# SciSharp/Gym.NET

Measured on AMD Instinct MI355X. Metric: env-steps/sec, higher is better.
Workload: dtype f32

## Files before the change

### gym.net_amd/csrc/envs.hpp

```cpp
#pragma once
#include <hip/hip_runtime.h>
#include <stdint.h>

#include "philox.hpp"

namespace gymnet {


typedef float f2 __attribute__((ext_vector_type(2)));
namespace vm {
__device__ __forceinline__ float splat(float, float v) { return v; }
__device__ __forceinline__ f2 splat(f2, float v) { return f2{v, v}; }
__device__ __forceinline__ float fma(float a, float b, float c) { return fmaf(a, b, c); }
__device__ __forceinline__ f2 fma(f2 a, f2 b, f2 c) { return __builtin_elementwise_fma(a, b, c); }
template <class T> __device__ __forceinline__ T fmak(float k, T b, T c) { return fma(splat(b, k), b, c); }
template <class T> __device__ __forceinline__ T fmac(T a, T b, float k) { return fma(a, b, splat(a, k)); }
}

__device__ __forceinline__ void sincos_quadrant(float s, float c, float n, float &s_out, float &c_out) {
    const uint32_t q = (uint32_t)(int)n;
    const uint32_t q30 = q << 30, q31 = q << 31;
    const bool odd = (int32_t)q31 < 0;
    const float ss = odd ? c : s, cc = odd ? s : c;
    s_out = __uint_as_float(__builtin_amdgcn_bitop3_b32(__float_as_uint(ss), q30, 0x80000000u, 0x78));
    c_out = __uint_as_float(__builtin_amdgcn_bitop3_b32(__float_as_uint(cc), q30 ^ q31, 0x80000000u, 0x78));
}

template <class T>
__device__ __forceinline__ void sincos_bounded(T x, T &s_out, T &c_out) {
    T n;
    const T xs = x * vm::splat(x, 0.636619772367581343f);
    if constexpr (sizeof(T) == sizeof(float)) n = rintf(xs);
    else n = T{rintf(xs.x), rintf(xs.y)};
    T r = vm::fmak(-1.5703125f, n, x);
    r = vm::fmak(-4.837512969970703125e-4f, n, r);
    r = vm::fmak(-7.54978995489188216e-8f, n, r);
    const T z = r * r;
    T ps = vm::fmac(vm::splat(z, -1.9515295891e-4f), z, 8.3321608736e-3f);
    ps = vm::fmac(ps, z, -1.6666654611e-1f);
    const T s = vm::fma(r * z, ps, r);
    T pc = vm::fmac(vm::splat(z, 2.443315711809948e-5f), z, -1.388731625493765e-3f);
    pc = vm::fmac(pc, z, 4.166664568298827e-2f);
    const T c = vm::fma(z * z, pc, vm::fmac(vm::splat(z, -0.5f), z, 1.0f));
    if constexpr (sizeof(T) == sizeof(float)) {
        sincos_quadrant(s, c, n, s_out, c_out);
    } else {
        float s0, c0, s1, c1;
        sincos_quadrant(s.x, c.x, n.x, s0, c0);
        sincos_quadrant(s.y, c.y, n.y, s1, c1);
        s_out = T{s0, s1};
        c_out = T{c0, c1};
    }
}

template <class T>
__device__ __forceinline__ void sincos_small(T x, T &s_out, T &c_out) {
    T n;
    const T xs = x * vm::splat(x, 0.636619772367581343f);
    if constexpr (sizeof(T) == sizeof(float)) n = rintf(xs);
    else n = T{rintf(xs.x), rintf(xs.y)};
    T r = vm::fmak(-0x1.921fap+0f, n, x);
    r = vm::fmak(-0x1.54442ep-20f, n, r);
    const T z = r * r;
    T ps = vm::fmac(vm::splat(z, -1.9515295891e-4f), z, 8.3321608736e-3f);
    ps = vm::fmac(ps, z, -1.6666654611e-1f);
    const T s = vm::fma(r * z, ps, r);
    T pc = vm::fmac(vm::splat(z, 2.443315711809948e-5f), z, -1.388731625493765e-3f);
    pc = vm::fmac(pc, z, 4.166664568298827e-2f);
    pc = vm::fmac(pc, z, -0.5f);
    const T c = vm::fmac(pc, z, 1.0f);
    if constexpr (sizeof(T) == sizeof(float)) {
        sincos_quadrant(s, c, n, s_out, c_out);
    } else {
        float s0, c0, s1, c1;
        sincos_quadrant(s.x, c.x, n.x, s0, c0);
        sincos_quadrant(s.y, c.y, n.y, s1, c1);
        s_out = T{s0, s1};
        c_out = T{c0, c1};
    }
}

constexpr float kSmallAngle = 0.785f;
__device__ __forceinline__ void sincos_tiny(float x, float &s_out, float &c_out) {
    const float z = x * x;
    float ps = fmaf(-1.9515295891e-4f, z, 8.3321608736e-3f);
    ps = fmaf(ps, z, -1.6666654611e-1f);
    s_out = fmaf(x * z, ps, x);
    float pc = fmaf(2.443315711809948e-5f, z, -1.388731625493765e-3f);
    pc = fmaf(pc, z, 4.166664568298827e-2f);
    c_out = fmaf(z * z, pc, fmaf(-0.5f, z, 1.0f));
}

template <bool BOUNDED = false>
__device__ __forceinline__ void sincos_f32(float x, float &s_out, float &c_out) {
    if constexpr (!BOUNDED) {
        if (__builtin_expect(fabsf(x) > 65536.0f, 0)) {
            sincosf(x, &s_out, &c_out);
            return;
        }
    }
    sincos_bounded<float>(x, s_out, c_out);
}
__device__ __forceinline__ float sin_f32(float x) { float s, c; sincos_f32(x, s, c); return s; }
__device__ __forceinline__ float cos_f32(float x) { float s, c; sincos_f32(x, s, c); return c; }

template <typename Dummy = void>
struct DivByTotalMass {
    static constexpr float C = 0.1f + 1.0f;
    static constexpr float ZH = 1.0f / C;
    static constexpr float ZL = (float)(1.0 / (double)C - (double)ZH);
    __device__ __forceinline__ static float apply(float x) { return fmaf(x, ZH, x * ZL); }
};

struct CartPole {
    static constexpr int S = 4;
    static constexpr int O = 4;
    static constexpr bool OBS_ALIASES_STATE = true;
    static constexpr bool HAS_SBD = true;
    static constexpr bool BOX_ACTION = false;
    static constexpr bool PACKED2 = false;
    static constexpr bool PIPE_LANES = false, PIPE_PAIRS = false;
    using Action = int32_t;
    using Real = float;
    static constexpr bool RESET_TAKES_KEY = false;
    static constexpr const char *NAME = "CartPole";
    static constexpr int32_t ACTION_N = 2;

    static constexpr float gravity = 9.8f;
    static constexpr float masspole = 0.1f;
    static constexpr float total_mass = 0.1f + 1.0f;
    static constexpr float length = 0.5f;
    static constexpr float polemass_length = 0.1f * 0.5f;
    static constexpr float force_mag = 10.0f;
    static constexpr float tau = 0.02f;
    static constexpr float theta_threshold = 0.20943951606750488f;
    static constexpr float x_threshold = 2.4f;

    __device__ __forceinline__ static float div_tm(float x) { return DivByTotalMass<>::apply(x); }

    static constexpr bool HAS_SMALL_ANGLE_PATH = true;
    static constexpr int ANGLE_ROW = 2;
    static constexpr float SMALL_ANGLE_BOUND = kSmallAngle;

    template <bool SMALL_ANGLE = false, bool AUTORESET = false>
    __device__ __forceinline__ static void step(float (&s)[S], Action a, float &reward, bool &done) {
        const float x = s[0], x_dot = s[1], theta = s[2], theta_dot = s[3];
        const float s_in[S] = {x, x_dot, theta, theta_dot};
        const float force = (a == 1) ? force_mag : -force_mag;
        float sintheta, costheta;
        if constexpr (SMALL_ANGLE) sincos_tiny(theta, sintheta, costheta);
        else sincos_f32(theta, sintheta, costheta);
        const float temp = div_tm(force + polemass_length * theta_dot * theta_dot * sintheta);
        const float thetaacc = (gravity * sintheta - costheta * temp)
                               / (length * (4.0f / 3.0f - div_tm(masspole * costheta * costheta)));
        const float xacc = temp - div_tm(polemass_length * thetaacc * costheta);
        const float nx = x + tau * x_dot;
        const float nx_dot = x_dot + tau * xacc;
        const float ntheta = theta + tau * theta_dot;
        const float ntheta_dot = theta_dot + tau * thetaacc;
        s[0] = nx; s[1] = nx_dot; s[2] = ntheta; s[3] = ntheta_dot;
        bool term[DONE_TERMS];
        done_terms_of_inputs(s_in, term);
        done = term[0] || term[1];
        reward = 1.0f;
    }

    static constexpr int DONE_TERMS = 2;
    __device__ __forceinline__ static void done_terms_of_inputs(const float (&s)[S], bool (&term)[DONE_TERMS]) {
        const double vx = __builtin_fma((double)tau, (double)s[1], (double)s[0]);
        const double vtheta = __builtin_fma((double)tau, (double)s[3], (double)s[2]);
        term[0] = __builtin_fabs(vx) > (double)x_threshold;
        term[1] = __builtin_fabs(vtheta) > (double)theta_threshold;
    }

    __device__ __forceinline__ static void reset(float (&s)[S], const PhiloxWords &r) {
#pragma unroll
        for (int k = 0; k < 4; ++k) s[k] = -0.05f + 0.1f * u01_24(r.w[k]);
    }

    __device__ __forceinline__ static void observe(const float (&s)[S], float (&o)[O]) {
#pragma unroll
        for (int k = 0; k < 4; ++k) o[k] = s[k];
    }
    __device__ __forceinline__ static void observe_fresh(const float (&s)[S], float (&o)[O]) { observe(s, o); }
    __device__ __forceinline__ static void step_observe(float (&s)[S], Action a, float &reward, bool &done, float (&o)[O]) {
        step(s, a, reward, done);
        observe(s, o);
    }
};

struct Pendulum {
    static constexpr int S = 2;
    static constexpr int O = 3;
    static constexpr bool OBS_ALIASES_STATE = false;
    static constexpr int OBS_ROW_OF_STATE[S] = {-1, 2};
    static constexpr bool HAS_SBD = false;
    static constexpr bool BOX_ACTION = true;
    static constexpr bool PACKED2 = false;
    static constexpr bool PIPE_LANES = false, PIPE_PAIRS = false;
    static constexpr bool HAS_SMALL_ANGLE_PATH = false;
    using Action = float;
    using Real = float;
    static constexpr bool RESET_TAKES_KEY = false;
    static constexpr const char *NAME = "Pendulum";
    static constexpr float ACTION_LOW = -2.0f, ACTION_HIGH = 2.0f;
    static constexpr float PI = 3.14159265358979323846f;

    __device__ __forceinline__ static float fmod_2pi(float a) {
        constexpr float m = 2.0f * PI, inv_m = 1.0f / m;
        const float ax = fabsf(a);
        if (__builtin_expect(!(ax < 4194304.0f * m), 0)) return fmodf(a, m);
        float q = truncf(ax * inv_m);
        float r = fmaf(-q, m, ax);
        q = r < 0.0f ? q - 1.0f : (r >= m ? q + 1.0f : q);
        r = fmaf(-q, m, ax);
        return copysignf(r, a);
    }

    __device__ __forceinline__ static float floored_mod_2pi(float a) {
        float r = fmod_2pi(a);
        if (r < 0.0f) r += 2.0f * PI;
        return r;
    }

    __device__ __forceinline__ static void step(float (&s)[S], Action a, float &reward, bool &done) {
        const float max_speed = 8.0f, max_torque = 2.0f, dt = 0.05f;
        const float th = s[0], thdot = s[1];
        const float u = a < -max_torque ? -max_torque : (a > max_torque ? max_torque : a);
        const float nrm = floored_mod_2pi(th + PI) - PI;
        const float costs = nrm * nrm + 0.1f * (thdot * thdot) + 0.001f * (u * u);
        float newthdot = thdot + (15.0f * sin_f32(th) + 3.0f * u) * dt;
        newthdot = newthdot < -max_speed ? -max_speed : (newthdot > max_speed ? max_speed : newthdot);
        const float newth = th + newthdot * dt;
        s[0] = newth; s[1] = newthdot;
        reward = -costs;
        done = false;
    }

    __device__ __forceinline__ static void reset(float (&s)[S], const PhiloxWords &r) {
        s[0] = -PI + (2.0f * PI) * u01_24(r.w[0]);
        s[1] = -1.0f + 2.0f * u01_24(r.w[1]);
    }

    __device__ __forceinline__ static void observe(const float (&s)[S], float (&o)[O]) {
        float sn, cs;
        sincos_f32(s[0], sn, cs);
        o[0] = cs; o[1] = sn; o[2] = s[1];
    }
    __device__ __forceinline__ static void observe_fresh(const float (&s)[S], float (&o)[O]) { observe(s, o); }
    __device__ __forceinline__ static void step_observe(float (&s)[S], Action a, float &reward, bool &done, float (&o)[O]) {
        step(s, a, reward, done);
        observe(s, o);
    }
};

struct MountainCar {
    static constexpr int S = 2;
    static constexpr int O = 2;
    static constexpr bool OBS_ALIASES_STATE = true;
    static constexpr bool HAS_SBD = false;
    static constexpr bool BOX_ACTION = false;
    static constexpr bool PACKED2 = false;
    static constexpr bool PIPE_LANES = false, PIPE_PAIRS = false;
    static constexpr bool HAS_SMALL_ANGLE_PATH = false;
    using Action = int32_t;
    using Real = float;
    static constexpr bool RESET_TAKES_KEY = false;
    static constexpr const char *NAME = "MountainCar";
    static constexpr int32_t ACTION_N = 3;

    __device__ __forceinline__ static void step(float (&s)[S], Action a, float &reward, bool &done) {
        float p = s[0], v = s[1];
        v += (float)(a - 1) * 0.001f + cos_f32(3.0f * p) * (-0.0025f);
        v = v < -0.07f ? -0.07f : (v > 0.07f ? 0.07f : v);
        p += v;
        p = p < -1.2f ? -1.2f : (p > 0.6f ? 0.6f : p);
        if (p == -1.2f && v < 0.0f) v = 0.0f;
        s[0] = p; s[1] = v;
        reward = -1.0f;
        done = p >= 0.5f && v >= 0.0f;
    }

    __device__ __forceinline__ static void reset(float (&s)[S], const PhiloxWords &r) {
        s[0] = -0.6f + 0.2f * u01_24(r.w[0]);
        s[1] = 0.0f;
    }

    __device__ __forceinline__ static void observe(const float (&s)[S], float (&o)[O]) { o[0] = s[0]; o[1] = s[1]; }
    __device__ __forceinline__ static void observe_fresh(const float (&s)[S], float (&o)[O]) { observe(s, o); }
    __device__ __forceinline__ static void step_observe(float (&s)[S], Action a, float &reward, bool &done, float (&o)[O]) {
        step(s, a, reward, done);
        observe(s, o);
    }
};

struct MountainCarContinuous {
    static constexpr int S = 2;
    static constexpr int O = 2;
    static constexpr bool OBS_ALIASES_STATE = true;
    static constexpr bool HAS_SBD = false;
    static constexpr bool BOX_ACTION = true;
    static constexpr bool PACKED2 = false;
    static constexpr bool PIPE_LANES = false, PIPE_PAIRS = false;
    static constexpr bool HAS_SMALL_ANGLE_PATH = false;
    using Action = float;
    using Real = float;
    static constexpr bool RESET_TAKES_KEY = false;
    static constexpr const char *NAME = "MountainCarContinuous";
    static constexpr float ACTION_LOW = -1.0f, ACTION_HIGH = 1.0f;
    static constexpr float GOAL = 0x1.cccccep-2f;

    __device__ __forceinline__ static void step(float (&s)[S], Action a, float &reward, bool &done) {
        float p = s[0], v = s[1];
        const float force = a < -1.0f ? -1.0f : (a > 1.0f ? 1.0f : a);
        v += force * 0.0015f - 0.0025f * cos_f32(3.0f * p);
        v = v < -0.07f ? -0.07f : (v > 0.07f ? 0.07f : v);
        p += v;
        p = p < -1.2f ? -1.2f : (p > 0.6f ? 0.6f : p);
        if (p == -1.2f && v < 0.0f) v = 0.0f;
// ... 161 lines not shown
```

### gym.net_amd/csrc/step_kernels.hpp

```cpp
#pragma once
#include "kernels.hpp"

#include <cstdio>
#include <type_traits>

#include "lanes.hpp"
#include "philox.hpp"

namespace gymnet {

__device__ __forceinline__ float abs_real(float x) { return fabsf(x); }
__device__ __forceinline__ double abs_real(double x) { return __builtin_fabs(x); }

template <class Env, bool UNIFORM_KEY = false>
__device__ __forceinline__ void draw_reset(typename Env::Real (&s)[Env::S], uint64_t key, uint64_t lane, uint64_t tick) {
    if constexpr (Env::RESET_TAKES_KEY) Env::reset(s, key, lane, tick);
    else Env::reset(s, lane_words<UNIFORM_KEY>(key, lane, tick));
}

template <class Env>
__device__ __forceinline__ constexpr bool state_row_own(int k) {
    if constexpr (Env::OBS_ALIASES_STATE) return true; else return Env::OBS_ROW_OF_STATE[k] < 0;
}
template <class Env>
__device__ __forceinline__ const typename Env::Real *state_row_src(const typename Env::Real *state, int64_t state_stride,
                                                                    const typename Env::Real *obs_in, int64_t obs_stride, int k) {
    if constexpr (Env::OBS_ALIASES_STATE) return state + k * state_stride;
    else return Env::OBS_ROW_OF_STATE[k] < 0 ? state + k * state_stride : obs_in + Env::OBS_ROW_OF_STATE[k] * obs_stride;
}

__device__ __forceinline__ uint32_t wave_shard() {
    return (uint32_t)((((int64_t)blockIdx.x * blockDim.x + threadIdx.x) >> 6) & (kShards - 1));
}

template <int VEC, class Args>
__device__ __forceinline__ void count_after_done(const Args &a, const bool (&after)[VEC]) {
    uint32_t total = 0;
#pragma unroll
    for (int j = 0; j < VEC; ++j) total += (uint32_t)__popcll(__ballot(after[j]));
    if (total && lane_id() == (uint32_t)(__ffsll((unsigned long long)__ballot(1)) - 1))
        atomicAdd(&a.after_done[wave_shard() * kAfterStride], (unsigned long long)total);
}

template <class Env, bool AUTORESET, bool SMALL_ANGLE = false>
__device__ __forceinline__ void advance_sublane(typename Env::Real (&sj)[Env::S], typename Env::Action act, int32_t &sbd, float &rw,
                                                bool &dn, bool &after, bool in_range, typename Env::Real (&oj)[Env::O]) {
    if constexpr (Env::HAS_SMALL_ANGLE_PATH) Env::template step<SMALL_ANGLE, AUTORESET>(sj, act, rw, dn);
    else if constexpr (Env::OBS_ALIASES_STATE) Env::step(sj, act, rw, dn);
    else Env::step_observe(sj, act, rw, dn, oj);
    if constexpr (!AUTORESET && Env::HAS_SBD) {
        if (dn) {
            if (sbd == -1) { sbd = 0; }
            else { after = in_range; sbd += 1; rw = 0.0f; }
        }
    }
}

template <class Env, int VEC>
__device__ __forceinline__ bool wave_angles_small(const typename Env::Real (&s)[Env::S][VEC]) {
    if constexpr (!Env::HAS_SMALL_ANGLE_PATH) return false;
    else {
        bool small = true;
#pragma unroll
        for (int j = 0; j < VEC; ++j) small = small && (abs_real(s[Env::ANGLE_ROW][j]) <= Env::SMALL_ANGLE_BOUND);
        return __ballot(!small) == 0;
    }
}

template <class Env, int VEC, bool AUTORESET, bool GUARD, bool PACK = true>
__device__ __forceinline__ void advance_all(typename Env::Real (&s)[Env::S][VEC], typename Env::Action (&act)[VEC], int32_t (&sbd)[VEC],
                                            float (&rw)[VEC], bool (&dn)[VEC], bool (&after)[VEC], typename Env::Real (&o)[Env::O][VEC],
                                            int64_t i0, int64_t n) {
    constexpr int S = Env::S, O = Env::O;
    using Real = typename Env::Real;
#ifndef GYMNET_PROBE_NO_PACK
    constexpr bool kPack = true;
#else
    constexpr bool kPack = false;
#endif
    if constexpr (Env::PACKED2 && VEC == 2 && kPack && PACK) {
        Env::step_observe_x2(s, act, rw, dn, o);
    } else {
        auto all_sublanes = [&](auto small_tag) {
#pragma unroll
            for (int j = 0; j < VEC; ++j) {
                Real sj[S], oj[O];
#pragma unroll
                for (int k = 0; k < S; ++k) sj[k] = s[k][j];
                advance_sublane<Env, AUTORESET, decltype(small_tag)::value>(sj, act[j], sbd[j], rw[j], dn[j], after[j], !GUARD || i0 + j < n, oj);
#pragma unroll
                for (int k = 0; k < S; ++k) s[k][j] = sj[k];
                if constexpr (!Env::OBS_ALIASES_STATE) {
#pragma unroll
                    for (int k = 0; k < O; ++k) o[k][j] = oj[k];
                }
            }
        };
        if constexpr (Env::HAS_SMALL_ANGLE_PATH) {
            if (wave_angles_small<Env, VEC>(s)) all_sublanes(std::true_type{});
            else all_sublanes(std::false_type{});
        } else {
            all_sublanes(std::false_type{});
        }
    }
}

template <class Env, class = void> struct has_done_of_inputs : std::false_type {};
template <class Env> struct has_done_of_inputs<Env, std::void_t<decltype(&Env::done_terms_of_inputs)>> : std::true_type {};

template <class Env, int VEC, bool AUTORESET>
__device__ __forceinline__ void advance_all_late_done(typename Env::Real (&s)[Env::S][VEC], typename Env::Action (&act)[VEC], float (&rw)[VEC],
                                                      bool (&dn)[VEC], uint64_t (&dmask)[VEC]) {
    constexpr int S = Env::S, O = Env::O;
    using Real = typename Env::Real;
    static_assert(Env::HAS_SMALL_ANGLE_PATH && Env::OBS_ALIASES_STATE && has_done_of_inputs<Env>::value, "see above");
    static_assert(AUTORESET || !Env::HAS_SBD, "the steps_beyond_done rule reads the flag inside the step");
    Real was[S][VEC];
#pragma unroll
    for (int k = 0; k < S; ++k)
#pragma unroll
        for (int j = 0; j < VEC; ++j) was[k][j] = s[k][j];
    auto all_sublanes = [&](auto small_tag) {
#pragma unroll
        for (int j = 0; j < VEC; ++j) {
            Real sj[S], oj[O];
            int32_t sbd_unused = 0;
            bool after_unused = false;
#pragma unroll
            for (int k = 0; k < S; ++k) sj[k] = s[k][j];
            advance_sublane<Env, AUTORESET, decltype(small_tag)::value>(sj, act[j], sbd_unused, rw[j], dn[j], after_unused, true, oj);
#pragma unroll
            for (int k = 0; k < S; ++k) s[k][j] = sj[k];
        }
    };
    if (wave_angles_small<Env, VEC>(s)) all_sublanes(std::true_type{});
    else all_sublanes(std::false_type{});
#pragma unroll
    for (int j = 0; j < VEC; ++j) {
        Real wj[S];
#pragma unroll
        for (int k = 0; k < S; ++k) wj[k] = was[k][j];
        bool term[Env::DONE_TERMS];
        Env::done_terms_of_inputs(wj, term);
        bool any = false;
        uint64_t m = 0;
#pragma unroll
        for (int q = 0; q < Env::DONE_TERMS; ++q) { any = any || term[q]; m |= __builtin_amdgcn_ballot_w64(term[q]); }
        dn[j] = any;
        dmask[j] = m;
    }
}

template <class Env, int VEC, bool LANE_SEEDS>
__device__ __forceinline__ void reset_pending(uint32_t pending, typename Env::Real (&s)[Env::S][VEC], typename Env::Real (&o)[Env::O][VEC],
                                              const StepArgsT<typename Env::Real> &a, int64_t i0, int64_t n, uint64_t tick) {
    constexpr int S = Env::S, O = Env::O;
    using Real = typename Env::Real;
    while (pending) {
        const int j = __ffs(pending) - 1;
        pending &= pending - 1;
        Real sj[S];
        bool drawn = false;
        if constexpr (LANE_SEEDS) {
            if (a.lane_seed) {
                draw_reset<Env, false>(sj, i0 + j < n ? a.lane_seed[i0 + j] : a.seed, a.lane_offset + (uint64_t)(i0 + j), tick);
                drawn = true;
            }
        }
        if (!drawn) draw_reset<Env, true>(sj, a.seed, a.lane_offset + (uint64_t)(i0 + j), tick);
        Real oj[O];
        if constexpr (!Env::OBS_ALIASES_STATE) Env::observe_fresh(sj, oj);
#pragma unroll
        for (int jj = 0; jj < VEC; ++jj) {
            if (jj == j) {
#pragma unroll
                for (int k = 0; k < S; ++k) s[k][jj] = sj[k];
                if constexpr (!Env::OBS_ALIASES_STATE) {
#pragma unroll
                    for (int k = 0; k < O; ++k) o[k][jj] = oj[k];
                }
            }
        }
    }
}

template <class Env>
constexpr bool has_split_reset() { return Env::RESET_TAKES_KEY && Env::OBS_ALIASES_STATE; }

__device__ __forceinline__ PhiloxWords neighbour_words(const PhiloxWords &w) {
    PhiloxWords o;
#pragma unroll
    for (int k = 0; k < 4; ++k) o.w[k] = (uint32_t)__builtin_amdgcn_mov_dpp((int)w.w[k], 0xB1, 0xF, 0xF, true);
    return o;
}

#ifdef GYMNET_PROBE_RESET_MASKED
constexpr bool kResetFullExec = false;
#else
constexpr bool kResetFullExec = true;
#endif

template <class Env>
struct ResetScratch {
    uint32_t slot[64];
    typename Env::Real draw[64][Env::S];
};

__device__ __forceinline__ void wave_lds_fence() {
    __builtin_amdgcn_fence(__ATOMIC_RELEASE, "wavefront");
    __builtin_amdgcn_wave_barrier();
    __builtin_amdgcn_fence(__ATOMIC_ACQUIRE, "wavefront");
}

template <class Env, int VEC, bool LANE_SEEDS>
__device__ __forceinline__ void reset_pending_wave(uint32_t pending, typename Env::Real (&s)[Env::S][VEC], const StepArgsT<typename Env::Real> &a,
                                                   int64_t i0, int64_t n, uint64_t tick, ResetScratch<Env> *sc) {
    constexpr int S = Env::S;
    using Real = typename Env::Real;
    static_assert(Env::OBS_ALIASES_STATE, "the compacted reset hands back the state only");
    const uint32_t lane = lane_id();
    uint32_t rank[VEC];
    uint32_t total = 0;
#pragma unroll
    for (int j = 0; j < VEC; ++j) {
        const uint64_t m = __ballot((pending >> j) & 1u);
        rank[j] = total + __builtin_amdgcn_mbcnt_hi((uint32_t)(m >> 32), __builtin_amdgcn_mbcnt_lo((uint32_t)m, 0u));
        total += (uint32_t)__popcll(m);
    }
    if (total == 0) return;
    const int64_t wave_i0 = i0 - (int64_t)lane * VEC;
    constexpr bool SPLIT = has_split_reset<Env>();
    const uint32_t active = (uint32_t)__popcll(__ballot(1));
    const uint32_t A = SPLIT ? active >> 1 : active;
    if constexpr (SPLIT) {
        if (A == 0) {
            Real o_unused[Env::O][VEC];
            reset_pending<Env, VEC, LANE_SEEDS>(pending, s, o_unused, a, i0, n, tick);
            return;
        }
    }
    for (uint32_t base = 0; base < total; base += A) {
#pragma unroll
        for (int j = 0; j < VEC; ++j)
            if (((pending >> j) & 1u) && rank[j] - base < A) sc->slot[rank[j] - base] = lane * VEC + (uint32_t)j;
        wave_lds_fence();
        if constexpr (SPLIT) {
            const uint32_t r = lane >> 1, call = lane & 1u;
            const bool draws = r < A && r < total - base;
            PhiloxWords w{};
            if (kResetFullExec || draws) {
                const uint32_t sl = sc->slot[draws ? r : 0u];
                const int64_t gl = wave_i0 + (int64_t)sl;
                uint64_t key = a.seed;
                if constexpr (LANE_SEEDS) {
                    if (a.lane_seed && gl < n) key = a.lane_seed[gl];
                }
                w = lane_words(Env::reset_call_key(key, call), a.lane_offset + (uint64_t)gl, tick);
            }
            const PhiloxWords other = neighbour_words(w);
            if ((kResetFullExec || draws) && call == 0) {
                Real sj[S];
                Env::reset_from_words(sj, w, other);
#pragma unroll
                for (int k = 0; k < S; ++k) sc->draw[r][k] = sj[k];
            }
        } else if (kResetFullExec || lane < total - base) {
            const uint32_t sl = sc->slot[lane < total - base ? lane : 0u];
            const int64_t gl = wave_i0 + (int64_t)sl;
            Real sj[S];
            bool drawn = false;
            if constexpr (LANE_SEEDS) {
                if (a.lane_seed) {
                    draw_reset<Env, false>(sj, gl < n ? a.lane_seed[gl] : a.seed, a.lane_offset + (uint64_t)gl, tick);
                    drawn = true;
                }
            }
            if (!drawn) draw_reset<Env, true>(sj, a.seed, a.lane_offset + (uint64_t)gl, tick);
#pragma unroll
            for (int k = 0; k < S; ++k) sc->draw[lane][k] = sj[k];
        }
        wave_lds_fence();
        Real got[VEC][S];
#pragma unroll
        for (int j = 0; j < VEC; ++j) {
            const uint32_t r = rank[j] - base;
#pragma unroll
            for (int k = 0; k < S; ++k) got[j][k] = sc->draw[r < A ? r : 0u][k];
        }
#pragma unroll
        for (int j = 0; j < VEC; ++j) {
            const bool mine = ((pending >> j) & 1u) && rank[j] - base < A;
#pragma unroll
            for (int k = 0; k < S; ++k) s[k][j] = mine ? got[j][k] : s[k][j];
        }
        wave_lds_fence();
    }
}

template <class Env, int VEC, bool LANE_SEEDS>
__device__ __forceinline__ void reset_finished_wave(const bool (&fin)[VEC], const uint64_t (&fmask)[VEC], typename Env::Real (&s)[Env::S][VEC], const StepArgsT<typename Env::Real> &a,
                                                    int64_t i0, int64_t wave_i0, int64_t n, uint64_t tick, ResetScratch<Env> *sc) {
    constexpr int S = Env::S;
    using Real = typename Env::Real;
    static_assert(Env::OBS_ALIASES_STATE && !has_split_reset<Env>(), "one-call resets that hand back the state only");
    const uint32_t lane = lane_id();
    uint32_t rank[VEC];
    uint32_t total = 0;
#pragma unroll
    for (int j = 0; j < VEC; ++j) {
        const uint64_t m = fmask[j];
        rank[j] = total + __builtin_amdgcn_mbcnt_hi((uint32_t)(m >> 32), __builtin_amdgcn_mbcnt_lo((uint32_t)m, 0u));
        total += (uint32_t)__popcll(m);
    }
    if (__builtin_expect(total == 0 || total > 64u || __ballot(1) != ~0ull, 0)) {
        if (total != 0) {
            uint32_t pending = 0;
#pragma unroll
            for (int j = 0; j < VEC; ++j) pending |= fin[j] ? (1u << j) : 0u;
            reset_pending_wave<Env, VEC, LANE_SEEDS>(pending, s, a, i0, n, tick, sc);
        }
        return;
    }
#pragma unroll
    for (int j = 0; j < VEC; ++j)
        if (fin[j]) sc->slot[rank[j]] = lane * VEC + (uint32_t)j;
    wave_lds_fence();
    {
        const uint32_t sl = sc->slot[lane < total ? lane : 0u];
        const int64_t gl = wave_i0 + (int64_t)sl;
        Real sj[S];
        bool drawn = false;
        if constexpr (LANE_SEEDS) {
            if (a.lane_seed) {
                draw_reset<Env, false>(sj, gl < n ? a.lane_seed[gl] : a.seed, a.lane_offset + (uint64_t)gl, tick);
                drawn = true;
            }
        }
        if (!drawn) draw_reset<Env, true>(sj, a.seed, a.lane_offset + (uint64_t)gl, tick);
#pragma unroll
        for (int k = 0; k < S; ++k) sc->draw[lane][k] = sj[k];
    }
    wave_lds_fence();
    Real got[VEC][S];
#pragma unroll
    for (int j = 0; j < VEC; ++j) {
#pragma unroll
        for (int k = 0; k < S; ++k) got[j][k] = sc->draw[rank[j] & 63u][k];
    }
#pragma unroll
    for (int j = 0; j < VEC; ++j) {
#pragma unroll
        for (int k = 0; k < S; ++k) s[k][j] = fin[j] ? got[j][k] : s[k][j];
    }
    wave_lds_fence();
}

template <int VEC>
__device__ __forceinline__ uint32_t rank_finished(const bool (&finished)[VEC], uint32_t (&off)[VEC]) {
    uint32_t total = 0;
#pragma unroll
    for (int j = 0; j < VEC; ++j) {
        const uint64_t m = __ballot(finished[j]);
        off[j] = total + __builtin_amdgcn_mbcnt_hi((uint32_t)(m >> 32), __builtin_amdgcn_mbcnt_lo((uint32_t)m, 0u));
        total += (uint32_t)__popcll(m);
    }
    return total;
}

template <class Env, int VEC>
__device__ __forceinline__ void append_done_records(const StepArgsT<typename Env::Real> &a, const bool (&finished)[VEC], int64_t i0,
                                                    const typename Env::Real (&s)[Env::S][VEC], const typename Env::Real (&o)[Env::O][VEC],
                                                    const float (&fin_ret)[VEC], const int32_t (&fin_len)[VEC], bool stats) {
    constexpr int S = Env::S, O = Env::O;
    const uint32_t lane = lane_id();
    uint32_t off[VEC];
    const uint32_t total = rank_finished<VEC>(finished, off);
    if (total) {
        const int leader = __ffsll((unsigned long long)__ballot(1)) - 1;
        const uint32_t shard = wave_shard();
        uint32_t base = 0;
        if ((int)lane == leader)
            base = atomicAdd(&a.done_count2[a.cparity * (kShards * kCountStride) + shard * kCountStride], total);
        base = __shfl(base, leader);
        const int64_t seg0 = (int64_t)shard * a.done_cap;
#pragma unroll
        for (int j = 0; j < VEC; ++j) {
            if (!finished[j]) continue;
            const int64_t pos = seg0 + base + off[j];
            a.done_list[pos] = (int32_t)(i0 + j);
            if (stats) { a.rec_ret[pos] = fin_ret[j]; a.rec_len[pos] = fin_len[j]; }
            if (a.rec_obs) {
#pragma unroll
                for (int k = 0; k < O; ++k)
                    a.rec_obs[((int64_t)shard * O + k) * a.done_cap + base + off[j]] = Env::OBS_ALIASES_STATE ? s[k < S ? k : 0][j] : o[k][j];
            }
        }
    }
}

template <class R>
__device__ __forceinline__ StepArgsT<R> hot_step_args(R *state, const void *action, int64_t n, int64_t state_stride, uint64_t *tick2, float *reward,
                                                      int32_t parity, const StepArgsT<R> &rest) {
    StepArgsT<R> a = rest;
    a.state = state; a.action = action; a.n = n; a.state_stride = state_stride; a.tick2 = tick2; a.reward = reward; a.parity = parity;
    return a;
}

template <class Env, int VEC>
struct LaneInputs {
    typename Env::Real s[Env::S][VEC];
    typename Env::Action act[VEC];
    int32_t sbd[VEC];
};

template <bool NT, class T>
__device__ __forceinline__ T load_elem(const T *p) { if constexpr (NT) return __builtin_nontemporal_load(p); else return *p; }

template <class T, int VEC, bool NT>
__device__ __forceinline__ void load_row_clamped(const T *__restrict__ p, int64_t i0, int64_t n, T (&v)[VEC]) {
#pragma unroll
    for (int j = 0; j < VEC; ++j) v[j] = load_elem<NT>(p + (i0 + j < n ? i0 + j : n - 1));
}

template <class Env, int VEC, bool AUTORESET, int NT>
__device__ __forceinline__ void load_inputs_clamped(const StepArgsT<typename Env::Real> &a, const int64_t i0, LaneInputs<Env, VEC> &in) {
    constexpr bool NT_SL = (NT & 1) != 0, NT_A = (NT & 4) != 0;
#pragma unroll
    for (int k = 0; k < Env::S; ++k)
        load_row_clamped<typename Env::Real, VEC, NT_SL>(state_row_src<Env>(a.state, a.state_stride, a.obs_in, a.obs_stride, k), i0, a.n, in.s[k]);
    if constexpr (Env::BOX_ACTION) load_row_clamped<float, VEC, NT_A>(static_cast<const float *>(a.action), i0, a.n, in.act);
    else load_row_clamped<int32_t, VEC, NT_A>(static_cast<const int32_t *>(a.action), i0, a.n, in.act);
#pragma unroll
    for (int j = 0; j < VEC; ++j) in.sbd[j] = 0;
    if constexpr (!AUTORESET && Env::HAS_SBD) load_row_clamped<int32_t, VEC, NT_SL>(a.sbd, i0, a.n, in.sbd);
}

template <class Env, int VEC, bool AUTORESET, int NT, bool GUARD>
__device__ __forceinline__ void load_inputs(const StepArgsT<typename Env::Real> &a, const int64_t i0, LaneInputs<Env, VEC> &in) {
    constexpr bool NT_SL = (NT & 1) != 0, NT_A = (NT & 4) != 0;
    if constexpr (GUARD) { load_inputs_clamped<Env, VEC, AUTORESET, NT>(a, i0, in); return; }
    const int64_t n = a.n;
#pragma unroll
    for (int k = 0; k < Env::S; ++k)
        load_row<typename Env::Real, VEC, NT_SL, GUARD>(state_row_src<Env>(a.state, a.state_stride, a.obs_in, a.obs_stride, k), i0, n, in.s[k]);
    if constexpr (Env::BOX_ACTION) load_f32<VEC, NT_A, GUARD>(static_cast<const float *>(a.action), i0, n, in.act);
    else load_i32<VEC, NT_A, GUARD>(static_cast<const int32_t *>(a.action), i0, n, in.act);
#pragma unroll
    for (int j = 0; j < VEC; ++j) in.sbd[j] = 0;
    if constexpr (!AUTORESET && Env::HAS_SBD) load_i32<VEC, NT_SL, GUARD>(a.sbd, i0, n, in.sbd);
}

template <class Env, int VEC, bool AUTORESET, bool EXTRAS, int NT, bool GUARD, int RESETF = 0, bool PACK = true>
__device__ __forceinline__ void advance_and_store(const StepArgsT<typename Env::Real> &a, const int64_t i0, const uint64_t tick,
                                                  LaneInputs<Env, VEC> &in, ResetScratch<Env> *sc = nullptr) {
    constexpr int S = Env::S, O = Env::O;
    using Real = typename Env::Real;
    constexpr bool NT_SS = (NT & 2) != 0, NT_O = (NT & 8) != 0;
    const int64_t n = a.n;
    Real (&s)[S][VEC] = in.s;
    typename Env::Action (&act)[VEC] = in.act;
    int32_t (&sbd)[VEC] = in.sbd;

    constexpr bool NT_SL = (NT & 1) != 0;
    float ep_ret[VEC], fin_ret[VEC];
    int32_t ep_len[VEC], fin_len[VEC];
    bool stats = false;
    if constexpr (EXTRAS) {
        stats = a.ep_ret != nullptr;
        if (stats) {
            if constexpr (GUARD) { load_row_clamped<float, VEC, NT_SL>(a.ep_ret, i0, n, ep_ret); load_row_clamped<int32_t, VEC, NT_SL>(a.ep_len, i0, n, ep_len); }
            else { load_f32<VEC, NT_SL, false>(a.ep_ret, i0, n, ep_ret); load_i32<VEC, NT_SL, false>(a.ep_len, i0, n, ep_len); }
        }
#pragma unroll
        for (int j = 0; j < VEC; ++j) { fin_ret[j] = 0.0f; fin_len[j] = 0; }
    }

    float reward[VEC];
    uint8_t done[VEC];
    bool finished[VEC];
    bool after[VEC];
#pragma unroll
    for (int j = 0; j < VEC; ++j) after[j] = false;
    Real o[O][VEC];
    uint32_t pending = 0;

    float rwv[VEC];
    bool dnv[VEC];
    advance_all<Env, VEC, AUTORESET, GUARD, PACK>(s, act, sbd, rwv, dnv, after, o, i0, n);

#pragma unroll
    for (int j = 0; j < VEC; ++j) {
        const float rw = rwv[j];
        uint8_t db = dnv[j] ? 1 : 0;
        if constexpr (EXTRAS) {
            if (stats) {
                ep_ret[j] += rw;
                ep_len[j] += 1;
                if (a.max_episode_steps > 0 && ep_len[j] >= a.max_episode_steps) db |= 2;
            }
        }
        const bool fin = db != 0;
        finished[j] = fin && (!GUARD || i0 + j < n);
        done[j] = db;
        reward[j] = rw;

        if constexpr (EXTRAS) {
            if (fin && a.final_obs && (!GUARD || i0 + j < n)) {
#pragma unroll
                for (int k = 0; k < O; ++k) a.final_obs[k * n + i0 + j] = Env::OBS_ALIASES_STATE ? s[k < S ? k : 0][j] : o[k][j];
            }
            if (stats && fin && (!GUARD || i0 + j < n)) {
                fin_ret[j] = ep_ret[j];
                fin_len[j] = ep_len[j];
                if (a.fin_ret) { a.fin_ret[i0 + j] = ep_ret[j]; a.fin_len[i0 + j] = ep_len[j]; }
                if constexpr (AUTORESET) { ep_ret[j] = 0.0f; ep_len[j] = 0; }
            }
        }

        if constexpr (AUTORESET) pending |= fin ? (1u << j) : 0u;
    }

    if constexpr (!AUTORESET && Env::HAS_SBD) count_after_done<VEC>(a, after);

    store_f32<VEC, NT_O, GUARD>(a.reward, i0, n, reward);
    store_u8<VEC, NT_O, GUARD>(a.done, i0, n, done);

    if constexpr (EXTRAS) {
        if (a.done_list) append_done_records<Env, VEC>(a, finished, i0, s, o, fin_ret, fin_len, stats);
    }

    if constexpr (AUTORESET && RESETF == 1) reset_pending_wave<Env, VEC, EXTRAS>(pending, s, a, i0, n, tick, sc);
    else if constexpr (AUTORESET) reset_pending<Env, VEC, EXTRAS>(pending, s, o, a, i0, n, tick);

#pragma unroll
    for (int k = 0; k < S; ++k)
        if (state_row_own<Env>(k)) store_row<Real, VEC, NT_SS, GUARD>(a.state_out + k * a.state_stride, i0, n, s[k]);
    if constexpr (!Env::OBS_ALIASES_STATE) {
#pragma unroll
        for (int k = 0; k < O; ++k) store_row<Real, VEC, NT_SS, GUARD>(a.obs + k * a.obs_stride, i0, n, o[k]);
    }
    if constexpr (!AUTORESET && Env::HAS_SBD) store_i32<VEC, NT_SS, GUARD>(a.sbd, i0, n, sbd);

    if constexpr (EXTRAS) {
        if (stats) { store_f32<VEC, NT_SS, GUARD>(a.ep_ret, i0, n, ep_ret); store_i32<VEC, NT_SS, GUARD>(a.ep_len, i0, n, ep_len); }
    }
}

template <class Env, int VEC, bool AUTORESET, bool EXTRAS, int NT, bool GUARD, int RESETF = 0>
__device__ __forceinline__ void step_body(const StepArgsT<typename Env::Real> &a, const int64_t i0, const uint64_t tick, ResetScratch<Env> *sc = nullptr) {
    LaneInputs<Env, VEC> in;
    load_inputs<Env, VEC, AUTORESET, NT, GUARD>(a, i0, in);
    advance_and_store<Env, VEC, AUTORESET, EXTRAS, NT, GUARD, RESETF>(a, i0, tick, in, sc);
}

template <class Env, bool AUTORESET, bool EXTRAS>
constexpr bool has_full_workgroup_body() {
    return AUTORESET && !EXTRAS && Env::HAS_SMALL_ANGLE_PATH && Env::OBS_ALIASES_STATE && !has_split_reset<Env>() && has_done_of_inputs<Env>::value;
}

template <class T>
__device__ __forceinline__ T *wg_row(T *row, const WgLanes &wg) { return wave_uniform(row + wg.first); }

template <class Env, int VEC, int NT, int RESETF>
__device__ __forceinline__ void step_body_wg(const StepArgsT<typename Env::Real> &a, const WgLanes wg, const uint64_t tick, ResetScratch<Env> *sc) {
    constexpr int S = Env::S;
    using Real = typename Env::Real;
    constexpr bool NT_SL = (NT & 1) != 0, NT_SS = (NT & 2) != 0, NT_A = (NT & 4) != 0, NT_O = (NT & 8) != 0;
    static_assert(!Env::BOX_ACTION && Env::OBS_ALIASES_STATE, "a discrete-action env whose observation is its state");
    const int64_t i0 = wg.first + (int64_t)wg.local;

    Real s[S][VEC];
    typename Env::Action act[VEC];
#pragma unroll
    for (int k = 0; k < S; ++k) load_row_wg<Real, VEC, NT_SL>(wg_row(static_cast<const Real *>(a.state) + k * a.state_stride, wg), wg.local, s[k]);
    load_row_wg<int32_t, VEC, NT_A>(wg_row(static_cast<const int32_t *>(a.action), wg), wg.local, act);

    float reward[VEC];
    bool finished[VEC];
    uint64_t fmask[VEC];
    advance_all_late_done<Env, VEC, true>(s, act, reward, finished, fmask);

    {
        const uint32_t local = reissued(wg.local);
        store_row_wg<float, VEC, NT_O>(wg_row(a.reward, wg), local, reward);
        uint32_t w = 0;
#pragma unroll
        for (int j = 0; j < VEC; ++j) w |= finished[j] ? (1u << (8 * j)) : 0u;
        store_done_word_wg<VEC, NT_O>(wg_row(a.done, wg), local, w);
    }

    if constexpr (RESETF == 1) {
        reset_finished_wave<Env, VEC, false>(finished, fmask, s, a, i0, wg.first + (int64_t)__builtin_amdgcn_readfirstlane(wg.local), a.n, tick, sc);
    } else {
        uint32_t pending = 0;
#pragma unroll
        for (int j = 0; j < VEC; ++j) pending |= finished[j] ? (1u << j) : 0u;
        Real o_unused[Env::O][VEC];
        reset_pending<Env, VEC, false>(pending, s, o_unused, a, i0, a.n, tick);
    }

    const uint32_t local = reissued(wg.local);
#pragma unroll
    for (int k = 0; k < S; ++k) store_row_wg<Real, VEC, NT_SS>(wg_row(a.state_out + k * a.state_stride, wg), local, s[k]);
}

template <class Env>
struct LaneOutputs { typename Env::Real s[Env::S], o[Env::O]; float reward; uint8_t done; int32_t sbd; };

template <class Env, bool AUTORESET>
__device__ __forceinline__ void compute_lane(const StepArgsT<typename Env::Real> &a, int64_t i, uint64_t tick, LaneInputs<Env, 1> &in,
                                             LaneOutputs<Env> &out) {
    constexpr int S = Env::S, O = Env::O;
    typename Env::Real o[O][1];
    float rw[1];
    bool dn[1], after[1] = {false};
    advance_all<Env, 1, AUTORESET, false>(in.s, in.act, in.sbd, rw, dn, after, o, i, a.n);
    if constexpr (!AUTORESET && Env::HAS_SBD) count_after_done<1>(a, after);
    if constexpr (AUTORESET) reset_pending<Env, 1, false>(dn[0] ? 1u : 0u, in.s, o, a, i, a.n, tick);
#pragma unroll
    for (int k = 0; k < S; ++k) out.s[k] = in.s[k][0];
#pragma unroll
    for (int k = 0; k < O; ++k) out.o[k] = o[k][0];
    out.reward = rw[0]; out.done = dn[0] ? 1 : 0; out.sbd = in.sbd[0];
}

template <class Env, bool AUTORESET, int NT>
__device__ __forceinline__ void store_lane(const StepArgsT<typename Env::Real> &a, int64_t i, const LaneOutputs<Env> &out) {
    constexpr bool NT_SS = (NT & 2) != 0, NT_O = (NT & 8) != 0;
    auto st = [](auto *p, auto v, bool nt) { if (nt) __builtin_nontemporal_store(v, p); else *p = v; };
    st(a.reward + i, out.reward, NT_O);
    if constexpr (NT_O) __builtin_nontemporal_store(out.done, a.done + i); else a.done[i] = out.done;
#pragma unroll
    for (int k = 0; k < Env::S; ++k)
        if (state_row_own<Env>(k)) st(a.state_out + k * a.state_stride + i, out.s[k], NT_SS);
    if constexpr (!Env::OBS_ALIASES_STATE) {
#pragma unroll
        for (int k = 0; k < Env::O; ++k) st(a.obs + k * a.obs_stride + i, out.o[k], NT_SS);
    }
    if constexpr (!AUTORESET && Env::HAS_SBD) a.sbd[i] = out.sbd;
}

template <class Env, int ITEMS, bool AUTORESET, int NT>
__global__ __launch_bounds__(256) void step_kernel_pipe(typename Env::Real *state, const void *action, int64_t n, int64_t state_stride, uint64_t *tick2,
                                                        float *reward, int32_t block, int32_t parity, const StepArgsT<typename Env::Real> rest) {
    const StepArgsT<typename Env::Real> a = hot_step_args(state, action, n, state_stride, tick2, reward, parity, rest);
    const uint64_t tick = a.tick2[a.parity];
    if (blockIdx.x == 0 && threadIdx.x == 0) a.tick2[a.parity ^ 1] = tick + 1;
    const int64_t T = (int64_t)gridDim.x * block;
    const int64_t i = (int64_t)blockIdx.x * block + threadIdx.x;
    LaneInputs<Env, 1> in[ITEMS];
#pragma unroll
    for (int k = 0; k < ITEMS; ++k) {
        const int64_t idx = i + k * T;
        load_inputs<Env, 1, AUTORESET, NT, false>(a, idx < a.n ? idx : a.n - 1, in[k]);
    }
#pragma unroll
    for (int k = 0; k < ITEMS; ++k) {
        LaneOutputs<Env> out;
        if (k == 0) {
#pragma unroll
            for (int c = 0; c < Env::S; ++c) asm volatile("" : "+v"(in[0].s[c][0]));
            asm volatile("" : "+v"(in[0].act[0]));
        }
        compute_lane<Env, AUTORESET>(a, i + k * T, tick, in[k], out);
        if (k == 0) {
#pragma unroll
            for (int kk = 1; kk < ITEMS; ++kk) {
#pragma unroll
                for (int c = 0; c < Env::S; ++c) asm volatile("" : "+v"(in[kk].s[c][0]), "+v"(out.s[Env::S - 1]));
                asm volatile("" : "+v"(in[kk].act[0]), "+v"(out.reward));
            }
        }
        if (i + k * T < a.n) store_lane<Env, AUTORESET, NT>(a, i + k * T, out);
    }
}

template <class Env>
struct DeferScratch {
    uint32_t slot[32];
    typename Env::Real draw[32][Env::S];
};

template <class Env, int PAIRS, class StateOf>
__device__ __forceinline__ void reset_group_deferred(uint32_t pending, StateOf s, const StepArgsT<typename Env::Real> &a, int64_t t_wave0,
                                                     int64_t T, int first_pair, uint64_t tick, DeferScratch<Env> *sc) {
    static_assert(Env::RESET_CALLS == 2 && 2 * PAIRS <= 8, "two lanes per reset; the slot word keeps 3 bits for the sub-lane position");
    constexpr int Q = 2 * PAIRS, S = Env::S;
    using Real = typename Env::Real;
    const uint32_t lane = lane_id();
    uint32_t rank[Q];
    uint32_t total = 0;
#pragma unroll
    for (int q = 0; q < Q; ++q) {
        const uint64_t m = __ballot((pending >> q) & 1u);
        rank[q] = total + __builtin_amdgcn_mbcnt_hi((uint32_t)(m >> 32), __builtin_amdgcn_mbcnt_lo((uint32_t)m, 0u));
        total += (uint32_t)__popcll(m);
    }
    for (uint32_t base = 0; base < total; base += 32) {
#pragma unroll
        for (int q = 0; q < Q; ++q)
            if (((pending >> q) & 1u) && rank[q] - base < 32u) sc->slot[rank[q] - base] = lane * 8u + (uint32_t)q;
        wave_lds_fence();
        const uint32_t r = lane >> 1, call = lane & 1u;
        const bool draws = r < total - base;
        PhiloxWords w{};
        if (kResetFullExec || draws) {
            const uint32_t sl = sc->slot[draws ? r : 0u];
            const uint32_t owner = sl >> 3, q = sl & 7u;
            const int64_t gl = ((t_wave0 + owner) + (int64_t)(first_pair + (int)(q >> 1)) * T) * 2 + (q & 1u);
            w = lane_words(Env::reset_call_key(a.seed, call), a.lane_offset + (uint64_t)gl, tick);
        }
        const PhiloxWords other = neighbour_words(w);
        if ((kResetFullExec || draws) && call == 0) {
            Real sj[S];
            Env::reset_from_words(sj, w, other);
#pragma unroll
            for (int k = 0; k < S; ++k) sc->draw[r][k] = sj[k];
        }
        wave_lds_fence();
        Real got[Q][S];
#pragma unroll
        for (int q = 0; q < Q; ++q) {
            const uint32_t rr = rank[q] - base;
#pragma unroll
            for (int k = 0; k < S; ++k) got[q][k] = sc->draw[rr < 32u ? rr : 0u][k];
        }
#pragma unroll
        for (int q = 0; q < Q; ++q) {
            const bool mine = ((pending >> q) & 1u) && rank[q] - base < 32u;
            Real (&sq)[S][2] = s(q / 2);
#pragma unroll
            for (int k = 0; k < S; ++k) sq[k][q % 2] = mine ? got[q][k] : sq[k][q % 2];
        }
        wave_lds_fence();
    }
}

template <class Env, int ITEMS, int NT, bool GUARD>
__device__ __forceinline__ void pipe2_split_body(const StepArgsT<typename Env::Real> &a, int64_t t, int64_t T, uint64_t tick, DeferScratch<Env> *sc) {
    using Real = typename Env::Real;
    constexpr bool NT_SS = (NT & 2) != 0, NT_O = (NT & 8) != 0;
    LaneInputs<Env, 2> in[ITEMS];
#pragma unroll
    for (int k = 0; k < ITEMS; ++k) {
        load_inputs<Env, 2, true, NT, GUARD>(a, (t + k * T) * 2, in[k]);
    }
    uint32_t pending = 0;
#pragma unroll
    for (int k = 0; k < ITEMS; ++k) {
        if (k == 0) {
#pragma unroll
// ... 858 lines not shown
```

Measured before the change: 161.6 billion.

## Split CartPole step into action-independent pre and post phases, draw resets ahead

Splits the CartPole step into an action-independent pre phase (sincos, divisor, next positions) and a cheap action-dependent post phase. Termination is computed from the inputs before the post phase, so the wave-wide reset draw (Philox plus LDS compaction) can be issued before the action-dependent arithmetic. Doing the draw first lets its latency overlap with the remaining math. The trade-offs are more live registers for the Pre structs and an empty asm barrier that pins the ordering. A probe macro can restore the old order.

```diff
diff --git a/gym.net_amd/csrc/envs.hpp b/gym.net_amd/csrc/envs.hpp
--- a/gym.net_amd/csrc/envs.hpp
+++ b/gym.net_amd/csrc/envs.hpp
@@ -165,6 +165,39 @@
         reward = 1.0f;
     }
 
+    struct Pre {
+        float x_dot, theta_dot;
+        float nx, ntheta;
+        float costheta;
+        float centrifugal;
+        float gsin;
+        float divisor;
+    };
+    template <bool SMALL_ANGLE = false>
+    __device__ __forceinline__ static void step_pre(const float (&s)[S], Pre &p) {
+        const float x = s[0], x_dot = s[1], theta = s[2], theta_dot = s[3];
+        float sintheta, costheta;
+        if constexpr (SMALL_ANGLE) sincos_tiny(theta, sintheta, costheta);
+        else sincos_f32(theta, sintheta, costheta);
+        p.centrifugal = polemass_length * theta_dot * theta_dot * sintheta;
+        p.gsin = gravity * sintheta;
+        p.divisor = length * (4.0f / 3.0f - div_tm(masspole * costheta * costheta));
+        p.costheta = costheta;
+        p.nx = x + tau * x_dot;
+        p.ntheta = theta + tau * theta_dot;
+        p.x_dot = x_dot;
+        p.theta_dot = theta_dot;
+    }
+    __device__ __forceinline__ static void step_post(const Pre &p, Action a, float (&s)[S], float &reward) { step_post(p, a == 1, s, reward); }
+    __device__ __forceinline__ static void step_post(const Pre &p, bool right, float (&s)[S], float &reward) {
+        const float force = right ? force_mag : -force_mag;
+        const float temp = div_tm(force + p.centrifugal);
+        const float thetaacc = (p.gsin - p.costheta * temp) / p.divisor;
+        const float xacc = temp - div_tm(polemass_length * thetaacc * p.costheta);
+        s[0] = p.nx; s[1] = p.x_dot + tau * xacc; s[2] = p.ntheta; s[3] = p.theta_dot + tau * thetaacc;
+        reward = 1.0f;
+    }
+
     static constexpr int DONE_TERMS = 2;
     __device__ __forceinline__ static void done_terms_of_inputs(const float (&s)[S], bool (&term)[DONE_TERMS]) {
         const double vx = __builtin_fma((double)tau, (double)s[1], (double)s[0]);
diff --git a/gym.net_amd/csrc/step_kernels.hpp b/gym.net_amd/csrc/step_kernels.hpp
--- a/gym.net_amd/csrc/step_kernels.hpp
+++ b/gym.net_amd/csrc/step_kernels.hpp
@@ -108,29 +108,22 @@
 template <class Env, class = void> struct has_done_of_inputs : std::false_type {};
 template <class Env> struct has_done_of_inputs<Env, std::void_t<decltype(&Env::done_terms_of_inputs)>> : std::true_type {};
 
-template <class Env, int VEC, bool AUTORESET>
-__device__ __forceinline__ void advance_all_late_done(typename Env::Real (&s)[Env::S][VEC], typename Env::Action (&act)[VEC], float (&rw)[VEC],
-                                                      bool (&dn)[VEC], uint64_t (&dmask)[VEC]) {
-    constexpr int S = Env::S, O = Env::O;
+template <class Env, class = void> struct has_split_step : std::false_type {};
+template <class Env> struct has_split_step<Env, std::void_t<typename Env::Pre>> : std::true_type {};
+
+template <class Env, int VEC>
+__device__ __forceinline__ void pre_all_late_done(const typename Env::Real (&s)[Env::S][VEC], typename Env::Pre (&pre)[VEC], bool (&dn)[VEC],
+                                                  uint64_t (&dmask)[VEC]) {
+    constexpr int S = Env::S;
     using Real = typename Env::Real;
-    static_assert(Env::HAS_SMALL_ANGLE_PATH && Env::OBS_ALIASES_STATE && has_done_of_inputs<Env>::value, "see above");
-    static_assert(AUTORESET || !Env::HAS_SBD, "the steps_beyond_done rule reads the flag inside the step");
-    Real was[S][VEC];
-#pragma unroll
-    for (int k = 0; k < S; ++k)
-#pragma unroll
-        for (int j = 0; j < VEC; ++j) was[k][j] = s[k][j];
+    static_assert(Env::HAS_SMALL_ANGLE_PATH && Env::OBS_ALIASES_STATE && has_done_of_inputs<Env>::value && has_split_step<Env>::value, "see above");
     auto all_sublanes = [&](auto small_tag) {
 #pragma unroll
         for (int j = 0; j < VEC; ++j) {
-            Real sj[S], oj[O];
-            int32_t sbd_unused = 0;
-            bool after_unused = false;
+            Real sj[S];
 #pragma unroll
             for (int k = 0; k < S; ++k) sj[k] = s[k][j];
-            advance_sublane<Env, AUTORESET, decltype(small_tag)::value>(sj, act[j], sbd_unused, rw[j], dn[j], after_unused, true, oj);
-#pragma unroll
-            for (int k = 0; k < S; ++k) s[k][j] = sj[k];
+            Env::template step_pre<decltype(small_tag)::value>(sj, pre[j]);
         }
     };
     if (wave_angles_small<Env, VEC>(s)) all_sublanes(std::true_type{});
@@ -139,7 +132,7 @@
     for (int j = 0; j < VEC; ++j) {
         Real wj[S];
 #pragma unroll
-        for (int k = 0; k < S; ++k) wj[k] = was[k][j];
+        for (int k = 0; k < S; ++k) wj[k] = s[k][j];
         bool term[Env::DONE_TERMS];
         Env::done_terms_of_inputs(wj, term);
         bool any = false;
@@ -148,6 +141,23 @@
         for (int q = 0; q < Env::DONE_TERMS; ++q) { any = any || term[q]; m |= __builtin_amdgcn_ballot_w64(term[q]); }
         dn[j] = any;
         dmask[j] = m;
+    }
+}
+
+template <class Env, int VEC>
+__device__ __forceinline__ void post_all(const typename Env::Pre (&pre)[VEC], const typename Env::Action (&act)[VEC], const uint64_t (&dmask)[VEC],
+                                         typename Env::Real (&s)[Env::S][VEC], float (&rw)[VEC]) {
+    constexpr int S = Env::S;
+    static_assert(std::is_same<typename Env::Action, int32_t>::value, "a discrete action");
+    int32_t one = 1;
+#pragma unroll
+    for (int jj = 0; jj < VEC; ++jj) asm volatile("" : "+s"(one) : "v"(pre[jj].divisor), "s"(dmask[jj]));
+#pragma unroll
+    for (int j = 0; j < VEC; ++j) {
+        typename Env::Real sj[S];
+        Env::step_post(pre[j], act[j] == one, sj, rw[j]);
+#pragma unroll
+        for (int k = 0; k < S; ++k) s[k][j] = sj[k];
     }
 }
 
@@ -297,33 +307,33 @@
     }
 }
 
+template <int VEC>
+struct FinishedRanks {
+    uint32_t rank[VEC];
+    uint32_t total;
+    bool single;
+};
+
 template <class Env, int VEC, bool LANE_SEEDS>
-__device__ __forceinline__ void reset_finished_wave(const bool (&fin)[VEC], const uint64_t (&fmask)[VEC], typename Env::Real (&s)[Env::S][VEC], const StepArgsT<typename Env::Real> &a,
-                                                    int64_t i0, int64_t wave_i0, int64_t n, uint64_t tick, ResetScratch<Env> *sc) {
+__device__ __forceinline__ void reset_finished_draw(const bool (&fin)[VEC], const uint64_t (&fmask)[VEC], const StepArgsT<typename Env::Real> &a,
+                                                    int64_t wave_i0, int64_t n, uint64_t tick, ResetScratch<Env> *sc, FinishedRanks<VEC> &fr) {
     constexpr int S = Env::S;
     using Real = typename Env::Real;
     static_assert(Env::OBS_ALIASES_STATE && !has_split_reset<Env>(), "one-call resets that hand back the state only");
     const uint32_t lane = lane_id();
-    uint32_t rank[VEC];
     uint32_t total = 0;
 #pragma unroll
     for (int j = 0; j < VEC; ++j) {
         const uint64_t m = fmask[j];
-        rank[j] = total + __builtin_amdgcn_mbcnt_hi((uint32_t)(m >> 32), __builtin_amdgcn_mbcnt_lo((uint32_t)m, 0u));
+        fr.rank[j] = total + __builtin_amdgcn_mbcnt_hi((uint32_t)(m >> 32), __builtin_amdgcn_mbcnt_lo((uint32_t)m, 0u));
         total += (uint32_t)__popcll(m);
     }
-    if (__builtin_expect(total == 0 || total > 64u || __ballot(1) != ~0ull, 0)) {
-        if (total != 0) {
-            uint32_t pending = 0;
-#pragma unroll
-            for (int j = 0; j < VEC; ++j) pending |= fin[j] ? (1u << j) : 0u;
-            reset_pending_wave<Env, VEC, LANE_SEEDS>(pending, s, a, i0, n, tick, sc);
-        }
-        return;
-    }
+    fr.total = total;
+    fr.single = !__builtin_expect(total == 0 || total > 64u || __ballot(1) != ~0ull, 0);
+    if (!fr.single) return;
 #pragma unroll
     for (int j = 0; j < VEC; ++j)
-        if (fin[j]) sc->slot[rank[j]] = lane * VEC + (uint32_t)j;
+        if (fin[j]) sc->slot[fr.rank[j]] = lane * VEC + (uint32_t)j;
     wave_lds_fence();
     {
         const uint32_t sl = sc->slot[lane < total ? lane : 0u];
@@ -341,11 +351,18 @@
         for (int k = 0; k < S; ++k) sc->draw[lane][k] = sj[k];
     }
     wave_lds_fence();
+}
+
+template <class Env, int VEC>
+__device__ __forceinline__ void reset_finished_take(const bool (&fin)[VEC], const FinishedRanks<VEC> &fr, typename Env::Real (&s)[Env::S][VEC],
+                                                    ResetScratch<Env> *sc) {
+    constexpr int S = Env::S;
+    using Real = typename Env::Real;
     Real got[VEC][S];
 #pragma unroll
     for (int j = 0; j < VEC; ++j) {
 #pragma unroll
-        for (int k = 0; k < S; ++k) got[j][k] = sc->draw[rank[j] & 63u][k];
+        for (int k = 0; k < S; ++k) got[j][k] = sc->draw[fr.rank[j] & 63u][k];
     }
 #pragma unroll
     for (int j = 0; j < VEC; ++j) {
@@ -353,6 +370,16 @@
         for (int k = 0; k < S; ++k) s[k][j] = fin[j] ? got[j][k] : s[k][j];
     }
     wave_lds_fence();
+}
+
+template <class Env, int VEC, bool LANE_SEEDS>
+__device__ __forceinline__ void reset_finished_rest(const bool (&fin)[VEC], const FinishedRanks<VEC> &fr, typename Env::Real (&s)[Env::S][VEC],
+                                                    const StepArgsT<typename Env::Real> &a, int64_t i0, int64_t n, uint64_t tick, ResetScratch<Env> *sc) {
+    if (fr.total == 0) return;
+    uint32_t pending = 0;
+#pragma unroll
+    for (int j = 0; j < VEC; ++j) pending |= fin[j] ? (1u << j) : 0u;
+    reset_pending_wave<Env, VEC, LANE_SEEDS>(pending, s, a, i0, n, tick, sc);
 }
 
 template <int VEC>
@@ -555,11 +582,18 @@
 
 template <class Env, bool AUTORESET, bool EXTRAS>
 constexpr bool has_full_workgroup_body() {
-    return AUTORESET && !EXTRAS && Env::HAS_SMALL_ANGLE_PATH && Env::OBS_ALIASES_STATE && !has_split_reset<Env>() && has_done_of_inputs<Env>::value;
+    return AUTORESET && !EXTRAS && Env::HAS_SMALL_ANGLE_PATH && Env::OBS_ALIASES_STATE && !has_split_reset<Env>() && has_done_of_inputs<Env>::value &&
+           has_split_step<Env>::value;
 }
 
 template <class T>
 __device__ __forceinline__ T *wg_row(T *row, const WgLanes &wg) { return wave_uniform(row + wg.first); }
+
+#ifdef GYMNET_PROBE_RESET_BEHIND_ACTION
+constexpr bool kResetDrawAhead = false;
+#else
+constexpr bool kResetDrawAhead = true;
+#endif
 
 template <class Env, int VEC, int NT, int RESETF>
 __device__ __forceinline__ void step_body_wg(const StepArgsT<typename Env::Real> &a, const WgLanes wg, const uint64_t tick, ResetScratch<Env> *sc) {
@@ -575,28 +609,47 @@
     for (int k = 0; k < S; ++k) load_row_wg<Real, VEC, NT_SL>(wg_row(static_cast<const Real *>(a.state) + k * a.state_stride, wg), wg.local, s[k]);
     load_row_wg<int32_t, VEC, NT_A>(wg_row(static_cast<const int32_t *>(a.action), wg), wg.local, act);
 
-    float reward[VEC];
+    typename Env::Pre pre[VEC];
     bool finished[VEC];
     uint64_t fmask[VEC];
-    advance_all_late_done<Env, VEC, true>(s, act, reward, finished, fmask);
-
-    {
+    pre_all_late_done<Env, VEC>(s, pre, finished, fmask);
+
+    float reward[VEC];
+    auto store_reward_done = [&] {
         const uint32_t local = reissued(wg.local);
         store_row_wg<float, VEC, NT_O>(wg_row(a.reward, wg), local, reward);
         uint32_t w = 0;
 #pragma unroll
         for (int j = 0; j < VEC; ++j) w |= finished[j] ? (1u << (8 * j)) : 0u;
         store_done_word_wg<VEC, NT_O>(wg_row(a.done, wg), local, w);
-    }
-
-    if constexpr (RESETF == 1) {
-        reset_finished_wave<Env, VEC, false>(finished, fmask, s, a, i0, wg.first + (int64_t)__builtin_amdgcn_readfirstlane(wg.local), a.n, tick, sc);
+    };
+
+    if constexpr (RESETF == 1 && kResetDrawAhead) {
+        FinishedRanks<VEC> fr;
+        reset_finished_draw<Env, VEC, false>(finished, fmask, a, wg.first + (int64_t)__builtin_amdgcn_readfirstlane(wg.local), a.n, tick, sc, fr);
+        if (fr.single) {
+            post_all<Env, VEC>(pre, act, fmask, s, reward);
+            reset_finished_take<Env, VEC>(finished, fr, s, sc);
+        } else {
+            post_all<Env, VEC>(pre, act, fmask, s, reward);
+            reset_finished_rest<Env, VEC, false>(finished, fr, s, a, wg.first + (int64_t)reissued(wg.local), a.n, tick, sc);
+        }
+        store_reward_done();
     } else {
-        uint32_t pending = 0;
-#pragma unroll
-        for (int j = 0; j < VEC; ++j) pending |= finished[j] ? (1u << j) : 0u;
-        Real o_unused[Env::O][VEC];
-        reset_pending<Env, VEC, false>(pending, s, o_unused, a, i0, a.n, tick);
+        post_all<Env, VEC>(pre, act, fmask, s, reward);
+        store_reward_done();
+        if constexpr (RESETF == 1) {
+            FinishedRanks<VEC> fr;
+            reset_finished_draw<Env, VEC, false>(finished, fmask, a, wg.first + (int64_t)__builtin_amdgcn_readfirstlane(wg.local), a.n, tick, sc, fr);
+            if (fr.single) reset_finished_take<Env, VEC>(finished, fr, s, sc);
+            else reset_finished_rest<Env, VEC, false>(finished, fr, s, a, i0, a.n, tick, sc);
+        } else {
+            uint32_t pending = 0;
+#pragma unroll
+            for (int j = 0; j < VEC; ++j) pending |= finished[j] ? (1u << j) : 0u;
+            Real o_unused[Env::O][VEC];
+            reset_pending<Env, VEC, false>(pending, s, o_unused, a, i0, a.n, tick);
+        }
     }
 
     const uint32_t local = reissued(wg.local);
```

Result: faster. 168.7 billion (median of 6 runs) (+4.4%).
